# hyperplane-lab/ACL-GAN

Measured on AMD Instinct MI355X. Metric: training images/sec at 256x256 (gen+dis step), higher is better.
Workload: dtype fp32

## Files before the change

### acl-gan_amd/csrc/conv_fast.hip

```cpp
#include "conv_fast_common.h"
#include <cstring>

namespace aclgan {
namespace {


constexpr int BK = 16;
constexpr int WG_MAX_CHUNK = 1024 + 16;
constexpr int LDK = BK + 4;

template <int T, bool KC>
__device__ __forceinline__ void read_frags(const float* __restrict__ tile, int ld, int base, int lane, float (&f)[T][8]) {
    const int l31 = lane & 31, kh = lane >> 5;
    if (KC) {
#pragma unroll
        for (int t = 0; t < T; ++t) {
            const f32x4* p = reinterpret_cast<const f32x4*>(tile + (base + t * 32 + l31) * LDK + kh * 8);
            const f32x4 a = p[0], b = p[1];
            f[t][0] = a.x; f[t][1] = a.y; f[t][2] = a.z; f[t][3] = a.w;
            f[t][4] = b.x; f[t][5] = b.y; f[t][6] = b.z; f[t][7] = b.w;
        }
    } else {
#pragma unroll
        for (int ks = 0; ks < 8; ++ks)
// ... 275 lines not shown
        const int n = n0 + nc * 4;
        bo[i] = krow * p.k * p.k * p.Ci + (n < p.Ci ? n : 0);
    }
    const int cpt = p.Co >> 4;
    int aoff[A_IT];
    f32x4 ra[A_IT], rb[B_IT];
    float za[A_IT];
    int f_tap = -1, tapoff = 0;

    auto fetch = [&](int kt) __attribute__((always_inline)) {
        const int tq = kt / cpt, cc = kt - tq * cpt;
        if (tq != f_tap) {
            f_tap = tq;
            const int t = compact ? tap_list[tq] : tq;
            const int ty = t / Tx, tx = t - ty * Tx;
            tapoff = ((cy + p.s * ty) * p.k + (cx + p.s * tx)) * p.Ci;
#pragma unroll
            for (int i = 0; i < A_IT; ++i) {
                const int oy = ay[i] - ty, ox = ax[i] - tx;
                const bool ok = (unsigned)oy < (unsigned)p.Ho && (unsigned)ox < (unsigned)p.Wo;
                bool okk = ok;
                if (p.band > 0) okk = ok && (oy < 2 || oy >= p.Ho - 2 || ox < 2 || ox >= p.Wo - 2);
                const int dpix = p.dyv ? (ab[i] * p.Hf + 2 * (oy + 1) + p.py) * p.Wf + 2 * (ox + 1) + p.px
                                       : (ab[i] * p.Ho + oy) * p.Wo + ox;
                aoff[i] = okk ? dpix * p.Co + q * 4 : -1;
            }
        }
#pragma unroll
        for (int i = 0; i < A_IT; ++i) {
            ra[i] = *reinterpret_cast<const f32x4*>(p.dy + (size_t)(aoff[i] < 0 ? 0 : aoff[i]) + cc * 16);
            za[i] = aoff[i] < 0 ? 0.f : 1.f;
        }
#pragma unroll
        for (int i = 0; i < B_IT; ++i)
            if ((BK * NVB) % NT == 0 || tid + i * NT < BK * NVB)
                rb[i] = *reinterpret_cast<const f32x4*>(p.w + (size_t)bo[i] + tapoff + (size_t)cc * 16 * p.k * p.k * p.Ci);
    };
    auto stage = [&](int buf, bool real) __attribute__((always_inline)) {
        float* a = As + buf * BM * LDK;
        float* b = Bs + buf * BK * LDB;
#pragma unroll
        for (int i = 0; i < A_IT; ++i) *reinterpret_cast<f32x4*>(a + (r0 + i * RP) * LDK + q * 4) = ra[i] * za[i];
#pragma unroll
        for (int i = 0; i < B_IT; ++i) {
            const int idx = tid + i * NT;
            if ((BK * NVB) % NT == 0 || idx < BK * NVB) {
                const int krow = idx / NVB, nc = idx - krow * NVB;
                *reinterpret_cast<f32x4*>(b + krow * LDB + nc * 4) = rb[i];
            }
        }
    };

    f32x16 acc[TM][TN];
#pragma unroll
    for (int i = 0; i < TM; ++i)
#pragma unroll
        for (int j = 0; j < TN; ++j)
#pragma unroll
            for (int r = 0; r < 16; ++r) acc[i][j][r] = 0.f;

    const int nk_all = ntap * cpt;
    const int nkz = (nk_all + p.ksplit - 1) / p.ksplit;
    const int kbeg = slice * nkz, nk = min(nkz, nk_all - kbeg);
    if (nk <= 0) return;
    ACL_GEMM_MAINLOOP(TM, TN, true, false, kbeg, nk, As, Bs, BM * LDK, BK * LDB, LDK, LDB, wm * TM * 32, wn * TN * 32);

    const int l31 = lane & 31, lh = lane >> 5;
#pragma unroll
    for (int j = 0; j < TN; ++j) {
        const int n = n0 + wn * TN * 32 + j * 32 + l31;
        if (n >= p.Ci) continue;
#pragma unroll
        for (int i = 0; i < TM; ++i) {
#pragma unroll
            for (int r = 0; r < 16; ++r) {
                const int of = ri_o[wm * TM * 32 + i * 32 + (r & 3) + 8 * (r >> 2) + 4 * lh];
                if (of >= 0) {
                    float* o = p.dxp + (size_t)of * p.Ci + n;
                    if (p.ksplit > 1 || (p.mode == 2 && !p.ringpad)) atomicAdd(o, acc[i][j][r]);
                    else if (p.accumulate) *o += acc[i][j][r];
                    else *o = acc[i][j][r];
                }
            }
        }
    }
}

template <int WM, int WN, int TM, int TN>
int launch_dgrad_fast(const ConvGeom& g, DgFP p, hipStream_t st) {
    constexpr int BM = WM * TM * 32, BN = WN * TN * 32;
    int mmax = 0;
    for (int cy = 0; cy < g.s; ++cy)
        for (int cx = 0; cx < g.s; ++cx) {
            const int ylo = g.p > cy ? (g.p - cy + g.s - 1) / g.s : 0, xlo = g.p > cx ? (g.p - cx + g.s - 1) / g.s : 0;
            const int yhi = std::min(p.Hc - 1, (g.p + g.Hi - 1 - cy) / g.s), xhi = std::min(p.Wc - 1, (g.p + g.Wi - 1 - cx) / g.s);
            int inner = (yhi - ylo + 1) * (xhi - xlo + 1);
            if (p.band > 0) inner = std::max(0, p.Hc - 2 * p.band) * std::max(0, p.Wc - 2 * p.band);
            const int rows = p.mode == 0 ? p.Hc * p.Wc : (p.mode == 1 ? inner : p.Hc * p.Wc - inner);
            mmax = std::max(mmax, g.B * rows);
        }
    if (mmax <= 0) return ACLGAN_OK;
    p.Mc = mmax;
    p.tiles_n = cdiv(g.Ci, BN);
    p.nwg = cdiv(p.Mc, BM) * p.tiles_n;
    const int nk_min = ((g.k + g.s - 1) / g.s) * ((g.k + g.s - 1) / g.s) * (g.Co / 16);
    const int nblk = p.nwg * g.s * g.s;
    p.ksplit = 1;
    const int nk_plan = (p.mode == 2 && p.band == 0) ? std::max(g.Co / 16, nk_min / ((g.k + g.s - 1) / g.s)) : nk_min;
    if (nblk < 128 && nk_plan >= 32 && !sw(SW_DETERMINISTIC) && !p.ringpad)
        p.ksplit = max(1, min(nk_plan / 8, 512 / nblk));
    if (p.ksplit > 1 && p.mode == 0) {
        hipError_t e = hipMemsetAsync(p.dxp, 0, conv_dgrad_scratch_bytes(g), st);
        if (e != hipSuccess) return hip_fail(e, "memset dxp");
    }
    if (p.ksplit > 1 && p.mode == 1 && !p.accumulate) {
        hipError_t e = hipMemsetAsync(p.dxp, 0, (size_t)g.B * g.Hi * g.Wi * g.Ci * sizeof(float), st);
        if (e != hipSuccess) return hip_fail(e, "memset dx");
    }
    hipLaunchKernelGGL((conv_dgrad_fast_kernel<WM, WN, TM, TN>), dim3(p.nwg, 1, g.s * g.s * p.ksplit), dim3(WM * WN * 64), 0, st, p);
    ACL_CHECK_LAUNCH("conv_dgrad_fast_kernel");
    return ACLGAN_OK;
}

template <int WM, int WN, int TM, int TN>
int launch_dgrad_halo(const ConvGeom& g, DgFP p, hipStream_t st) {
    if (p.band == 0 && !p.ringpad && g.k == 3 && g.s == 1 && g.Ci % 128 == 0 && WM == 2 && WN == 2 && TM == 2 && TN == 2)
        return launch_dgrad_fast<2, 2, 1, 2>(g, p, st);
    return launch_dgrad_fast<WM, WN, TM, TN>(g, p, st);
}

template <int WM, int WN, int TM, int TN>
int dgrad_fast_all(const ConvGeom& g, DgFP p, float* dxp, float* dx, int accumulate, bool* direct, hipStream_t st) {
    if (g.up == 0 && dx != nullptr && (!sw(SW_DETERMINISTIC) || g.p == 0 || (dxp && conv_wino_ok(g)))) {
        *direct = true;
        p.dxp = dx; p.accumulate = accumulate;
        p.mode = 1;
        int rc = (dxp && conv_wino_ok(g)) ? conv_dgrad_wino_interior(g, p.dy, p.w, dx, accumulate, dxp, st)
             : (dxp && conv_s2k4_wino_ok(g, 1)) ? conv_dgrad_s2k4_wino_interior(g, p.dy, p.w, dx, accumulate, dxp, st)
                                      : launch_dgrad_fast<WM, WN, TM, TN>(g, p, st);
        if (rc) return rc;
        if (g.p > 0 && sw(SW_DETERMINISTIC)) {
            hipError_t e = hipMemsetAsync(dxp, 0, (size_t)g.B * g.Hp * g.Wp * g.Ci * sizeof(float), st);
            if (e != hipSuccess) return hip_fail(e, "memset padded grid");
            p.mode = 2; p.ringpad = 1; p.dxp = dxp; p.accumulate = 0;
            rc = launch_dgrad_fast<WM, WN, TM, TN>(g, p, st);
            if (rc) return rc;
            return conv_fold(g, dxp, dx, 1, st);
        }
        if (g.p > 0) { p.mode = 2; rc = launch_dgrad_halo<WM, WN, TM, TN>(g, p, st); }
        return rc;
    }
    *direct = false;
    p.dxp = dxp; p.mode = 0; p.accumulate = 0;
    return launch_dgrad_fast<WM, WN, TM, TN>(g, p, st);
}


template <int WM, int WN, int TM, int TN, bool ST>
__global__ void __launch_bounds__(WM * WN * 64) conv_wgrad_fast_kernel(WgFP p) {
    constexpr int BM = WM * TM * 32, BN = WN * TN * 32, NT = WM * WN * 64;
    constexpr int LDA = BM + 4, LDB = BN + 4, MVA = BM / 4, NVB = BN / 4;
    constexpr int A_IT = (BK * MVA + NT - 1) / NT, B_IT = (BK * NVB + NT - 1) / NT;
    __shared__ __attribute__((aligned(16))) float smem[2 * BK * (LDA + LDB)];
    float* As = smem;
    float* Bs = smem + 2 * BK * LDA;

    const int tid = threadIdx.x, lane = tid & 63, wave = tid >> 6;
    const int wm = wave / WN, wn = wave % WN;
    const int tile = xcd_map(blockIdx.x, p.nwg);
    const int m0 = (tile / p.tiles_n) * BM, n0 = (tile % p.tiles_n) * BN;
    const int pbeg = blockIdx.z * p.chunk;
    const int pend = min(p.P, pbeg + p.chunk);
    if (pbeg >= pend) return;
    const int phase = p.phases ? (int)blockIdx.y : 0;
    float* dwbase = p.dw + (size_t)phase * p.Co * p.Kn + (size_t)blockIdx.z * p.dw_zs;
    const int py = phase >> 1, px = phase & 1;

    __shared__ int4 pinfo[WG_MAX_CHUNK];
    const int st_tap = n0 / p.Ci, st_ky = st_tap / p.k, st_kx = st_tap - st_ky * p.k;
    for (int i = tid; i < pend - pbeg + BK; i += NT) {
        int b, oy, ox;
        wg_coord(p, min(pbeg + i, pend - 1), b, oy, ox);
        const int dyp = p.phases ? (b * p.Hf + 2 * (oy + 1) + py) * p.Wf + 2 * (ox + 1) + px : (b * p.Ho + oy) * p.Wo + ox;
        if (ST) {
            const int iy = refl(oy * p.s - p.p + st_ky, p.Hu) >> p.up, ix = refl(ox * p.s - p.p + st_kx, p.Wu) >> p.up;
            pinfo[i] = make_int4(b * p.Hi * p.Wi + iy * p.Wi + ix, 0, 0, dyp);
        } else {
            pinfo[i] = make_int4(oy * p.s - p.p, ox * p.s - p.p, b * p.Hi * p.Wi, dyp);
        }
    }
    __syncthreads();

    int a_m[A_IT], a_kr[A_IT];
#pragma unroll
    for (int i = 0; i < A_IT; ++i) {
        const int idx = tid + i * NT;
        a_kr[i] = idx / MVA;
        const int m = m0 + (idx - a_kr[i] * MVA) * 4;
        a_m[i] = m < p.Co ? m : 0;
    }
    int b_kr[B_IT], b_ci[B_IT], b_ky[B_IT], b_kx[B_IT];
#pragma unroll
    for (int i = 0; i < B_IT; ++i) {
        const int idx = tid + i * NT;
        b_kr[i] = idx / NVB;
        int n = n0 + (idx - b_kr[i] * NVB) * 4;
        if (n >= p.Kn) n = 0;
        const int tap = n / p.Ci;
        b_ci[i] = n - tap * p.Ci; b_ky[i] = tap / p.k; b_kx[i] = tap - b_ky[i] * p.k;
    }
    f32x4 ra[A_IT], rb[B_IT];
    float za[A_IT];
    const bool do_bias = p.db != nullptr && (tile % p.tiles_n) == 0;
    f32x4 bsum[A_IT];
#pragma unroll
    for (int i = 0; i < A_IT; ++i) bsum[i] = (f32x4){0.f, 0.f, 0.f, 0.f};

    auto fetch = [&](int kt) __attribute__((always_inline)) {
        const int pb = kt * BK;
#pragma unroll
        for (int i = 0; i < A_IT; ++i) {
            if ((BK * MVA) % NT != 0 && tid + i * NT >= BK * MVA) continue;
            const int pi = pb + a_kr[i];
            ra[i] = *reinterpret_cast<const f32x4*>(p.dy + (size_t)pinfo[pi].w * p.Co + a_m[i]);
            za[i] = pbeg + pi < pend ? 1.f : 0.f;
        }
#pragma unroll
        for (int i = 0; i < B_IT; ++i) {
            if ((BK * NVB) % NT != 0 && tid + i * NT >= BK * NVB) continue;
            if (ST) {
                rb[i] = *reinterpret_cast<const f32x4*>(p.x + (size_t)pinfo[pb + b_kr[i]].x * p.Ci + b_ci[i]);
            } else {
                const int4 pi = pinfo[pb + b_kr[i]];
                const int iy = refl(pi.x + b_ky[i], p.Hu) >> p.up;
                const int ix = refl(pi.y + b_kx[i], p.Wu) >> p.up;
                rb[i] = *reinterpret_cast<const f32x4*>(p.x + (size_t)(pi.z + iy * p.Wi + ix) * p.Ci + b_ci[i]);
            }
        }
    };
    auto stage = [&](int buf, bool real) __attribute__((always_inline)) {
        float* a = As + buf * BK * LDA;
        float* b = Bs + buf * BK * LDB;
#pragma unroll
        for (int i = 0; i < A_IT; ++i) {
            const int idx = tid + i * NT;
            if ((BK * MVA) % NT == 0 || idx < BK * MVA) {
                const f32x4 v = ra[i] * za[i];
                *reinterpret_cast<f32x4*>(a + a_kr[i] * LDA + (idx - a_kr[i] * MVA) * 4) = v;
                bsum[i] += v * (real ? 1.f : 0.f);
            }
        }
#pragma unroll
        for (int i = 0; i < B_IT; ++i) {
            const int idx = tid + i * NT;
            if ((BK * NVB) % NT == 0 || idx < BK * NVB) *reinterpret_cast<f32x4*>(b + b_kr[i] * LDB + (idx - b_kr[i] * NVB) * 4) = rb[i];
        }
    };

    f32x16 acc[TM][TN];
#pragma unroll
    for (int i = 0; i < TM; ++i)
#pragma unroll
        for (int j = 0; j < TN; ++j)
#pragma unroll
            for (int r = 0; r < 16; ++r) acc[i][j][r] = 0.f;

    ACL_GEMM_MAINLOOP(TM, TN, false, false, 0, (pend - pbeg + BK - 1) / BK, As, Bs, BK * LDA, BK * LDB, LDA, LDB, wm * TM * 32, wn * TN * 32);

    if (do_bias) {
        float* red = smem;
#pragma unroll
        for (int i = 0; i < A_IT; ++i) {
            const int idx = tid + i * NT;
            if ((BK * MVA) % NT == 0 || idx < BK * MVA) *reinterpret_cast<f32x4*>(red + a_kr[i] * BM + (idx - a_kr[i] * MVA) * 4) = bsum[i];
        }
        __syncthreads();
        if (tid < BM && m0 + tid < p.Co) {
            float t = 0.f;
#pragma unroll
            for (int r = 0; r < BK; ++r) t += red[r * BM + tid];
            atomicAdd(p.db + (size_t)blockIdx.z * p.db_zs + m0 + tid, t);
        }
    }
    const int l31 = lane & 31, lh = lane >> 5;
#pragma unroll
    for (int j = 0; j < TN; ++j) {
        const int n = n0 + wn * TN * 32 + j * 32 + l31;
        if (n >= p.Kn) continue;
#pragma unroll
        for (int i = 0; i < TM; ++i) {
#pragma unroll
            for (int r = 0; r < 16; ++r) {
                const int m = m0 + wm * TM * 32 + i * 32 + (r & 3) + 8 * (r >> 2) + 4 * lh;
                if (m < p.Co) {
                    atomicAdd(dwbase + (size_t)m * p.Kn + n, acc[i][j][r]);
                }
            }
        }
    }
}

constexpr int WGKC_TARGET = 768;

template <int WM, int WN, int TM, int TN>
__global__ void __launch_bounds__(WM * WN * 64) conv_wgrad_kc_kernel(WgFP pk, WgPartX xp) {
    constexpr int BM = WM * TM * 32, BN = WN * TN * 32, NT = WM * WN * 64;
    WgFP p = pk;
    if (pk.fsl) {
        const long long f = blockIdx.y;
        p.x += (pk.fsx_mod ? f % pk.fsx_mod : f) * pk.fs_x; p.dy += f * pk.fs_dy;
    }
    static_assert(BM % 64 == 0 && BN % 64 == 0 && BM + BN <= NT, "one staging unit (4 channels x 4 pixels) per thread, wave-uniform roles");
    constexpr int CH = 1024;
    __shared__ __attribute__((aligned(16))) float smem[2 * (BM + BN) * LDK];
    __shared__ int2 pinfo[CH + BK];
    float* As = smem;
    float* Bs = smem + 2 * BM * LDK;

    const int tid = threadIdx.x, lane = tid & 63, wave = tid >> 6;
    const int wm = wave / WN, wn = wave % WN;
    const int tile = xcd_map(blockIdx.x, p.nwg);
    const int m0 = (tile / p.tiles_n) * BM, n0 = (tile % p.tiles_n) * BN;
    const int pbeg = blockIdx.z * p.chunk;
    const int pend = min(p.P, pbeg + p.chunk);
    const int phase = (p.phases || p.fsl) ? (int)blockIdx.y : 0;
    float* dwbase = p.dw + (size_t)phase * p.Co * p.Kn;
    const int py = phase >> 1, px = phase & 1;
    const int st_tap = n0 / p.Ci, st_ky = st_tap / p.k, st_kx = st_tap - st_ky * p.k;

    const bool isA = tid < BM, isB = !isA && tid < BM + BN;
    const int u = isA ? tid : tid - BM;
    const int ncg = (isA ? BM : BN) >> 2;
    const int cg = u % ncg, pg = u / ncg;
    const float* src = isA ? p.dy : p.x;
    const int cstride = isA ? p.Co : p.Ci;
    const int chan = isA ? m0 + 4 * cg : (n0 - st_tap * p.Ci) + 4 * cg;
    float* mytile = isA ? As : Bs;
    const int tstride = (isA ? BM : BN) * LDK;
    f32x4 rr[4];
    float zm[4];
    const bool do_bias = p.db != nullptr && (tile % p.tiles_n) == 0;
    f32x4 bsum = {0.f, 0.f, 0.f, 0.f};

    f32x16 acc[TM][TN];
#pragma unroll
    for (int i = 0; i < TM; ++i)
#pragma unroll
        for (int j = 0; j < TN; ++j)
#pragma unroll
            for (int r = 0; r < 16; ++r) acc[i][j][r] = 0.f;

    for (int cb = pbeg; cb < pend; cb += CH) {
        const int ce = min(pend, cb + CH);
        for (int i = tid; i < ce - cb + BK; i += NT) {
            int b, oy, ox;
            wg_coord(p, min(cb + i, ce - 1), b, oy, ox);
            const int dyp = p.phases ? (b * p.Hf + 2 * (oy + 1) + py) * p.Wf + 2 * (ox + 1) + px : (b * p.Ho + oy) * p.Wo + ox;
            const int iy = refl(oy * p.s - p.p + st_ky, p.Hu) >> p.up, ix = refl(ox * p.s - p.p + st_kx, p.Wu) >> p.up;
            pinfo[i] = make_int2(b * p.Hi * p.Wi + iy * p.Wi + ix, dyp);
        }
        __syncthreads();

        auto fetch = [&](int kt) __attribute__((always_inline)) {
            const int pb = kt * BK + 4 * pg;
            if (isA || isB) {
#pragma unroll
                for (int j = 0; j < 4; ++j) {
                    const int2 pi = pinfo[pb + j];
                    rr[j] = *reinterpret_cast<const f32x4*>(src + (size_t)(isA ? pi.y : pi.x) * cstride + chan);
                    zm[j] = cb + pb + j < ce ? 1.f : 0.f;
                }
            }
        };
        auto stage = [&](int buf, bool real) __attribute__((always_inline)) {
            if (isA || isB) {
                float* t = mytile + buf * tstride;
                f32x4 v[4];
#pragma unroll
                for (int j = 0; j < 4; ++j) v[j] = rr[j] * zm[j];
                if (isA) {
                    const float on = real ? 1.f : 0.f;
#pragma unroll
                    for (int j = 0; j < 4; ++j) bsum += v[j] * on;
                }
#pragma unroll
                for (int c = 0; c < 4; ++c) {
                    const f32x4 k4 = {v[0][c], v[1][c], v[2][c], v[3][c]};
                    *reinterpret_cast<f32x4*>(t + (c * ncg + cg) * LDK + 4 * pg) = k4;
                }
            }
        };
        ACL_GEMM_MAINLOOP(TM, TN, true, true, 0, (ce - cb + BK - 1) / BK, As, Bs, BM * LDK, BN * LDK, LDK, LDK, wm * TM * 32, wn * TN * 32);
    }

    const bool partial = xp.part != nullptr;
    if (do_bias) {
        float* red = smem;
        if (isA) *reinterpret_cast<f32x4*>(red + pg * BM + 4 * cg) = bsum;
        __syncthreads();
        if (tid < BM) {
            const float t = red[tid] + red[BM + tid] + red[2 * BM + tid] + red[3 * BM + tid];
            if (partial) xp.part_b[((size_t)blockIdx.z * xp.ny + phase) * p.Co + m0 + tid] = t;
            else p.db[m0 + tid] += t;
        }
    }
    const int l31 = lane & 31, lh = lane >> 5;
    constexpr int MQ = BM / 4, NQ = BN / 4;
    if (partial) {
        float* pt = xp.part + (((size_t)blockIdx.z * xp.ny + phase) * p.nwg + tile) * (BM * BN);
#pragma unroll
        for (int j = 0; j < TN; ++j)
#pragma unroll
            for (int i = 0; i < TM; ++i)
#pragma unroll
                for (int r = 0; r < 16; ++r) {
                    const int rw = wm * TM * 32 + i * 32 + (r & 3) + 8 * (r >> 2) + 4 * lh;
                    pt[rw * BN + wn * TN * 32 + j * 32 + l31] = acc[i][j][r];
                }
        return;
    }
#pragma unroll
    for (int j = 0; j < TN; ++j) {
        const int cr = wn * TN * 32 + j * 32 + l31;
        const int n = n0 + 4 * (cr % NQ) + cr / NQ;
#pragma unroll
        for (int i = 0; i < TM; ++i) {
#pragma unroll
            for (int r = 0; r < 16; ++r) {
                const int rw = wm * TM * 32 + i * 32 + (r & 3) + 8 * (r >> 2) + 4 * lh;
                const int m = m0 + 4 * (rw % MQ) + rw / MQ;
                dwbase[(size_t)m * p.Kn + n] += acc[i][j][r];
            }
        }
    }
}

bool wgrad_kc_ok(const ConvGeom& g) {
    return !sw(SW_NOWGKC) && g.Co % 64 == 0 && g.Ci % 64 == 0;
}

template <int WM, int WN, int TM, int TN>
int launch_wgrad_kc(const ConvGeom& g, WgFP p, void* part, hipStream_t st) {
    constexpr int BM = WM * TM * 32, BN = WN * TN * 32;
    const int ny = p.fsl ? p.fsl : (p.phases ? 4 : 1);
    const WgPlan q = wgrad_plan(g.Co, p.Ci, p.Kn, p.P, ny, BK, WGKC_TARGET);
    if (q.BM != BM || q.BN != BN) { set_error("wgrad_kc: tile plan mismatch"); return ACLGAN_EINVAL; }
    p.tiles_n = q.tiles_n; p.nwg = q.nwg; p.chunk = q.chunk;
    WgPartX xp;
    xp.ny = ny; xp.part = nullptr; xp.part_b = nullptr;
    const bool use_part = q.splits > 1 || ny > 1;
    if (use_part) {
        if (!part) { set_error("wgrad_kc: %d slices need the scratch buffer", q.splits); return ACLGAN_EINVAL; }
        xp.part = (float*)part;
        xp.part_b = xp.part + (size_t)q.splits * ny * q.nwg * BM * BN;
    }
    hipLaunchKernelGGL((conv_wgrad_kc_kernel<WM, WN, TM, TN>), dim3(p.nwg, ny, q.splits), dim3(WM * WN * 64), 0, st, p, xp);
    ACL_CHECK_LAUNCH("conv_wgrad_kc_kernel");
    if (use_part) {
        const int64_t n = (int64_t)ny * g.Co * (p.Kn / 4);
        hipLaunchKernelGGL(wgrad_finish_kernel, dim3((int)std::min<int64_t>(cdiv64(n, 256), 4096)), dim3(256), 0, st, p, xp, BM, BN, q.splits);
        ACL_CHECK_LAUNCH("wgrad_finish_kernel");
    }
    return ACLGAN_OK;
}
int launch_wgrad_kc_any(const ConvGeom& g, const WgFP& p, void* part, hipStream_t st) {
    if (g.Co % 128 == 0 && p.Ci % 128 == 0) return launch_wgrad_kc<2, 2, 2, 2>(g, p, part, st);
    if (g.Co % 128 == 0) return launch_wgrad_kc<2, 2, 2, 1>(g, p, part, st);
    if (p.Ci % 128 == 0) return launch_wgrad_kc<2, 2, 1, 2>(g, p, part, st);
    return launch_wgrad_kc<2, 2, 1, 1>(g, p, part, st);
}

template <int WM, int WN, int TM, int TN>
int launch_wgrad_fast(const ConvGeom& g, WgFP p, hipStream_t st, void* det_part = nullptr) {
    constexpr int BM = WM * TM * 32, BN = WN * TN * 32;
    p.tiles_n = cdiv(p.Kn, BN);
    p.nwg = cdiv(g.Co, BM) * p.tiles_n;
    const int target = 1536;
    const int ny = p.phases ? 4 : 1;
    int splits = max(1, target / (p.nwg * ny));
    splits = max(1, min(splits, cdiv(p.P, 256)));
    splits = max(splits, cdiv(p.P, 1024));
    p.chunk = cdiv(cdiv(p.P, splits), 16) * 16;
    splits = cdiv(p.P, p.chunk);
    float* dw_out = p.dw; float* db_out = p.db;
    const int64_t ndw = (int64_t)ny * g.Co * p.Kn;
    if (det_part != nullptr && splits > 1) {
        hipError_t e = hipMemsetAsync(det_part, 0, (size_t)splits * (ndw + g.Co) * sizeof(float), st);
        if (e != hipSuccess) return hip_fail(e, "memset wgrad slices");
        p.dw = (float*)det_part; p.dw_zs = ndw;
        if (p.db) { p.db = (float*)det_part + (size_t)splits * ndw; p.db_zs = g.Co; }
    }
    if (p.Ci % BN == 0) hipLaunchKernelGGL((conv_wgrad_fast_kernel<WM, WN, TM, TN, true>), dim3(p.nwg, ny, splits), dim3(WM * WN * 64), 0, st, p);
    else hipLaunchKernelGGL((conv_wgrad_fast_kernel<WM, WN, TM, TN, false>), dim3(p.nwg, ny, splits), dim3(WM * WN * 64), 0, st, p);
    ACL_CHECK_LAUNCH("conv_wgrad_fast_kernel");
    if (p.dw_zs) {
        int rc = reduce_slices_ordered(p.dw, ndw, splits, dw_out, st);
        if (rc) return rc;
        if (db_out) { rc = reduce_slices_ordered(p.db, g.Co, splits, db_out, st); if (rc) return rc; }
    }
    return ACLGAN_OK;
}
size_t wgrad_fast_det_bytes(const ConvGeom& g, int Kn, int P, int ny) {
    const int nwg = cdiv(g.Co, 128) * cdiv(Kn, 128);
    int splits = std::max(1, 1536 / (nwg * ny));
    splits = std::max(1, std::min(splits, cdiv(P, 256)));
    splits = std::max(splits, cdiv(P, 1024)) + 1;
    return (size_t)splits * ((size_t)ny * g.Co * Kn + g.Co) * sizeof(float) + 256;
}


template <int WM, int WN, int TM, int TN>
int up5_fwd_t(const ConvGeom& g, const float* x, const float* w, const float* bias, float* y, float* wp, hipStream_t st, float* keepV) {
    const int64_t nm = (int64_t)4 * g.Co * 9 * (g.Ci / 4);
    if (!(conv_up5_wino_ok(g) && wino_u_cached(w, conv_up5_wino_u_variant(g, 0, keepV != nullptr)))) {
        hipLaunchKernelGGL(up5_merge_kernel, dim3((int)std::min<int64_t>(cdiv64(nm, 256), 2048)), dim3(256), 0, st, w, wp, g.Co, g.Ci);
        ACL_CHECK_LAUNCH("up5_merge_kernel");
    }
    FwdFP p;
    p.fsl = 0; p.fsx_mod = 0; p.fs_x = p.fs_w = p.fs_y = 0; p.w16 = nullptr; p.x16 = nullptr;
    p.x = x; p.w = wp; p.bias = bias; p.y = y;
    p.Hi = g.Hi; p.Wi = g.Wi; p.Ci = g.Ci; p.Ho = g.Hi - 2; p.Wo = g.Wi - 2; p.Co = g.Co; p.k = 3; p.s = 1; p.p = 0;
    p.up = 0; p.Hu = g.Hi; p.Wu = g.Wi; p.M = g.B * p.Ho * p.Wo; p.K = 9 * g.Ci; p.act = g.act; p.tiles_n = 0; p.nwg = 0; p.nkz = 0;
    p.B = g.B; p.ring = 0; p.phases = 1; p.Hf = g.Ho; p.Wf = g.Wo; p.part = nullptr; p.rows = 0;
    ConvGeom gp = g;
    gp.M = p.M; gp.K = p.K;
    char* wino_scr = (char*)wp + up5_merged_bytes(g) + ((fwd_partial_bytes(g, 2, BK) + 255) & ~(size_t)255);
    if (keepV && !conv_up5_wino_ok(g)) { set_error("conv_fwd: this layer does not keep a Winograd input transform"); return ACLGAN_EINVAL; }
    int rc = conv_up5_wino_ok(g) ? conv_up5_wino_fwd_phases(g, x, wp, bias, y, wino_scr, st, keepV, w) : launch_fwd_fast<WM, WN, TM, TN>(gp, p, st);
    if (rc) return rc;
    p.w = w;
    p.Hi = g.Hi; p.Wi = g.Wi; p.Ho = g.Ho; p.Wo = g.Wo; p.k = 5; p.s = 1; p.p = 2; p.up = 1; p.Hu = g.Hu; p.Wu = g.Wu;
    p.M = g.M; p.K = g.K; p.ring = 2; p.phases = 0;
    p.part = (float*)((char*)wp + up5_merged_bytes(g));
    return launch_fwd_fast<WM, WN, TM, TN>(g, p, st);
}

template <int WM, int WN, int TM, int TN>
int up5_wgrad_t(const ConvGeom& g, const float* x, const float* dy, float* dw, float* db, float* dwp, hipStream_t st, const float* haveV) {
    const size_t nb = (size_t)4 * g.Co * 9 * g.Ci * sizeof(float);
    hipError_t e = hipMemsetAsync(dwp, 0, nb, st);
    if (e != hipSuccess) return hip_fail(e, "memset dwp");
    const bool kc = wgrad_kc_ok(g);
    void* part = (char*)dwp + up5_dwp_bytes(g);
    WgFP p;
    p.fsl = 0; p.fsx_mod = 0; p.fs_x = p.fs_dy = 0;
    p.x = x; p.dy = dy; p.dw = dwp; p.db = db;
    p.Hi = g.Hi; p.Wi = g.Wi; p.Ci = g.Ci; p.Ho = g.Hi - 2; p.Wo = g.Wi - 2; p.Co = g.Co; p.k = 3; p.s = 1; p.p = 0;
    p.up = 0; p.Hu = g.Hi; p.Wu = g.Wi; p.P = g.B * p.Ho * p.Wo; p.Kn = 9 * g.Ci; p.chunk = 0; p.tiles_n = 0; p.nwg = 0;
    p.B = g.B; p.ring = 0; p.phases = 1; p.Hf = g.Ho; p.Wf = g.Wo;
    int rc;
    if (kc && conv_up5_wino_wgrad_scratch_bytes(g)) {
        void* wino_scr = (char*)dwp + ((wgrad_part_scratch(g, BK, WGKC_TARGET) + 255) & ~(size_t)255);
        rc = conv_up5_wino_wgrad_phases(g, x, dy, dwp, db, wino_scr, st, haveV);
    } else rc = kc ? launch_wgrad_kc_any(g, p, part, st) : launch_wgrad_fast<WM, WN, TM, TN>(g, p, st);
    if (rc) return rc;
    const int64_t ns = (int64_t)g.Co * 25 * (g.Ci / 4);
    hipLaunchKernelGGL(up5_scatter_kernel, dim3((int)std::min<int64_t>(cdiv64(ns, 256), 2048)), dim3(256), 0, st, dwp, dw, g.Co, g.Ci);
    ACL_CHECK_LAUNCH("up5_scatter_kernel");
    p.dw = dw;
    p.Hi = g.Hi; p.Wi = g.Wi; p.Ho = g.Ho; p.Wo = g.Wo; p.k = 5; p.s = 1; p.p = 2; p.up = 1; p.Hu = g.Hu; p.Wu = g.Wu;
    p.ring = 2; p.phases = 0; p.Kn = g.K;
    p.P = g.B * (g.Ho * g.Wo - (g.Ho - 4) * (g.Wo - 4));
    return kc ? launch_wgrad_kc_any(g, p, part, st) : launch_wgrad_fast<WM, WN, TM, TN>(g, p, st);
}

template <int WM, int WN, int TM, int TN>
int up5_dgrad_t(const ConvGeom& g, const float* dy, const float* w, float* dx, int accumulate, float* wp, hipStream_t st) {
    const int64_t nm = (int64_t)4 * g.Co * 9 * (g.Ci / 4);
    if (!(conv_up5_wino_ok(g) && wino_u_cached(w, conv_up5_wino_u_variant(g, 1, false)))) {
        hipLaunchKernelGGL(up5_merge_kernel, dim3((int)std::min<int64_t>(cdiv64(nm, 256), 2048)), dim3(256), 0, st, w, wp, g.Co, g.Ci);
        ACL_CHECK_LAUNCH("up5_merge_kernel");
    }
    ConvGeom gv = g;
    gv.k = 3; gv.s = 1; gv.p = 0; gv.up = 0; gv.Hu = g.Hi; gv.Wu = g.Wi; gv.Hp = g.Hi; gv.Wp = g.Wi;
    gv.Ho = g.Hi - 2; gv.Wo = g.Wi - 2; gv.M = g.B * gv.Ho * gv.Wo; gv.K = 9 * g.Ci;
    DgFP p;
    p.dy = dy; p.dxp = dx;
    p.Ho = gv.Ho; p.Wo = gv.Wo; p.Co = g.Co; p.Ci = g.Ci; p.k = 3; p.s = 1; p.Hp = g.Hi; p.Wp = g.Wi;
    p.Hc = g.Hi; p.Wc = g.Wi; p.Mc = 0; p.tiles_n = 0; p.nwg = 0; p.ksplit = 1;
    p.mode = 1; p.pad = 0; p.B = g.B; p.Hi = g.Hi; p.Wi = g.Wi;
    p.dyv = 1; p.Hf = g.Ho; p.Wf = g.Wo; p.band = 0; p.upshift = 0; p.Hd = g.Hi; p.Wd = g.Wi;
    if (conv_up5_wino_ok(g)) {
        const int rc = conv_up5_wino_dgrad_phases(g, dy, wp, dx, accumulate, (char*)wp + up5_merged_bytes(g), st, w);
        if (rc) return rc;
    } else for (int ph = 0; ph < 4; ++ph) {
        p.w = wp + (size_t)ph * g.Co * 9 * g.Ci;
        p.py = ph >> 1; p.px = ph & 1;
        p.accumulate = (ph > 0 || accumulate) ? 1 : 0;
        const int rc = launch_dgrad_fast<WM, WN, TM, TN>(gv, p, st);
        if (rc) return rc;
    }
    p.w = w;
    p.Ho = g.Ho; p.Wo = g.Wo; p.k = 5; p.s = 1; p.Hp = g.Hp; p.Wp = g.Wp; p.Hc = g.Hp; p.Wc = g.Wp;
    p.mode = 2; p.accumulate = 1; p.pad = 2; p.Hi = g.Hu; p.Wi = g.Wu;
    p.dyv = 0; p.band = 6; p.upshift = 1; p.Hd = g.Hi; p.Wd = g.Wi;
    if (sw(SW_DETERMINISTIC)) {
        float* dxp = (float*)((char*)wp + up5_merged_bytes(g));
        hipError_t e = hipMemsetAsync(dxp, 0, (size_t)g.B * g.Hp * g.Wp * g.Ci * sizeof(float), st);
        if (e != hipSuccess) return hip_fail(e, "memset padded grid");
        p.ringpad = 1; p.dxp = dxp; p.accumulate = 0;
        const int rc = launch_dgrad_fast<WM, WN, TM, TN>(g, p, st);
        if (rc) return rc;
        return conv_fold(g, dxp, dx, 1, st);
    }
    return launch_dgrad_fast<WM, WN, TM, TN>(g, p, st);
}


}

size_t conv_up5_scratch_bytes(const ConvGeom& g) {
    return up5_eligible(g) ? (size_t)4 * g.Co * 9 * g.Ci * sizeof(float) : 0;
}
size_t conv_up5_dgrad_scratch_bytes(const ConvGeom& g) {
    if (sw(SW_NOFAST) || !up5_eligible(g)) return 0;
    const size_t padded = sw(SW_DETERMINISTIC) ? (size_t)g.B * g.Hp * g.Wp * g.Ci * sizeof(float) : 0;
    return up5_merged_bytes(g) + std::max(conv_up5_wino_dgrad_scratch_bytes(g), padded);
}
size_t conv_wgrad_fast_scratch_bytes(const ConvGeom& g) {
    if (sw(SW_NOFAST)) return 0;
    if (wgrad_kc_ok(g) && conv_wino_ok(g)) return conv_wgrad_wino_scratch_bytes(g);
    if (wgrad_kc_ok(g)) return ((wgrad_part_scratch(g, BK, WGKC_TARGET) + 255) & ~(size_t)255) + (up5_eligible(g) ? conv_up5_wino_wgrad_scratch_bytes(g) : 0);
    if (sw(SW_DETERMINISTIC)) return wgrad_fast_det_bytes(g, g.K, g.M, 1);
    return conv_up5_scratch_bytes(g);
}
size_t conv_fwd_fast_scratch_bytes(const ConvGeom& g) {
    if (sw(SW_NOFAST)) return 0;
    if (conv_wino_ok(g)) return conv_wino_scratch_bytes(g);
    if (up5_eligible(g)) return up5_merged_bytes(g) + ((fwd_partial_bytes(g, 2, BK) + 255) & ~(size_t)255) + conv_up5_wino_fwd_scratch_bytes(g);
    return std::max(fwd_partial_bytes(g, 0, BK), conv_s2k4_wino_scratch_bytes(g));
}

int conv_up5_fwd(const ConvGeom& g, const float* x, const float* w, const float* bias, float* y, void* scratch, hipStream_t st, float* keepV) {
    if (sw(SW_NOFAST) || !up5_eligible(g) || !scratch) return ACLGAN_EUNSUPPORTED;
    if (g.Co > 64) return up5_fwd_t<2, 2, 2, 2>(g, x, w, bias, y, (float*)scratch, st, keepV);
    if (g.Co > 32) return up5_fwd_t<4, 1, 2, 2>(g, x, w, bias, y, (float*)scratch, st, keepV);
    return up5_fwd_t<4, 1, 2, 1>(g, x, w, bias, y, (float*)scratch, st, keepV);
}

int conv_up5_dgrad(const ConvGeom& g, const float* dy, const float* w, float* dx, int accumulate, void* scratch, hipStream_t st) {
    if (sw(SW_NOFAST) || !up5_eligible(g) || !scratch) return ACLGAN_EUNSUPPORTED;
    if (sw(SW_NOUP5DGRAD)) return ACLGAN_EUNSUPPORTED;
    if (g.Ci > 64) return up5_dgrad_t<2, 2, 2, 2>(g, dy, w, dx, accumulate, (float*)scratch, st);
    if (g.Ci > 32) return up5_dgrad_t<4, 1, 2, 2>(g, dy, w, dx, accumulate, (float*)scratch, st);
    return up5_dgrad_t<4, 1, 2, 1>(g, dy, w, dx, accumulate, (float*)scratch, st);
}

int conv_up5_wgrad(const ConvGeom& g, const float* x, const float* dy, float* dw, float* db, void* scratch, hipStream_t st, const float* haveV) {
    if (sw(SW_NOFAST) || !up5_eligible(g) || !scratch || !dw) return ACLGAN_EUNSUPPORTED;
    if (sw(SW_DETERMINISTIC) && !wgrad_kc_ok(g)) return ACLGAN_EUNSUPPORTED;
    if (g.Co > 64) return up5_wgrad_t<2, 2, 2, 2>(g, x, dy, dw, db, (float*)scratch, st, haveV);
    if (g.Co > 32) return up5_wgrad_t<2, 2, 1, 2>(g, x, dy, dw, db, (float*)scratch, st, haveV);
    return up5_wgrad_t<1, 4, 1, 2>(g, x, dy, dw, db, (float*)scratch, st, haveV);
}

int gemm_slices_f32(const float* A, const float* Bm, float* Cm, int T, int K, int N, int nslices, int a_mod, hipStream_t st) {
    if (K % 16 != 0 || T <= 0 || N <= 0) { set_error("gemm_slices_f32: bad shape"); return ACLGAN_EINVAL; }
    FwdFP p;
    p.part = nullptr; p.rows = 0; p.w16 = nullptr; p.x16 = nullptr;
    p.x = A; p.w = Bm; p.bias = nullptr; p.y = Cm;
    p.Hi = T; p.Wi = 1; p.Ci = K; p.Ho = T; p.Wo = 1; p.Co = N; p.k = 1; p.s = 1; p.p = 0;
    p.up = 0; p.Hu = T; p.Wu = 1; p.M = T; p.K = K; p.act = ACLGAN_ACT_NONE; p.tiles_n = 0; p.nwg = 0; p.nkz = K / BK;
    p.B = 1; p.ring = 0; p.phases = 0; p.Hf = 0; p.Wf = 0;
    p.fsl = nslices; p.fsx_mod = a_mod; p.fs_x = (long long)T * K; p.fs_w = (long long)N * K; p.fs_y = (long long)T * N;
    if (N > 64) {
        p.tiles_n = cdiv(N, 128); p.nwg = cdiv(T, 64) * p.tiles_n;
        hipLaunchKernelGGL((conv_fwd_fast_kernel<2, 2, 1, 2, 4>), dim3(p.nwg, nslices, 1), dim3(256), 0, st, p);
    } else if (N > 32) {
        p.tiles_n = cdiv(N, 64); p.nwg = cdiv(T, 256) * p.tiles_n;
        hipLaunchKernelGGL((conv_fwd_fast_kernel<4, 1, 2, 2>), dim3(p.nwg, nslices, 1), dim3(256), 0, st, p);
    } else {
        p.tiles_n = cdiv(N, 32); p.nwg = cdiv(T, 256) * p.tiles_n;
        hipLaunchKernelGGL((conv_fwd_fast_kernel<4, 1, 2, 1>), dim3(p.nwg, nslices, 1), dim3(256), 0, st, p);
    }
    ACL_CHECK_LAUNCH("conv_fwd_fast_kernel(gemm slices)");
    return ACLGAN_OK;
}

int conv_fwd_stats_chunk(const ConvGeom& g) {
    if (sw(SW_NOSTATFUSE) || sw(SW_NOFAST) || g.Ci % 16 != 0 || g.act != ACLGAN_ACT_NONE) return 0;
    if (conv_wino_ok(g)) return 16;
    return (g.Ho % 4 == 0 && g.Wo % 4 == 0 && conv_s2k4_wino_ok(g, 0)) ? 16 : 0;
}
size_t conv_fwd_keep_bytes(const ConvGeom& g) {
    if (sw(SW_NOKEEPV) || sw(SW_NOFAST) || !wgrad_kc_ok(g)) return 0;
    if (up5_eligible(g)) return conv_up5_wino_wgrad_scratch_bytes(g) ? conv_up5_wino_keep_bytes(g) : 0;
    if (g.Ci % 16 != 0 || !conv_wino_ok(g) || !conv_wgrad_wino_scratch_bytes(g)) return 0;
    return conv_wino_keep_bytes(g);
}
int conv_fwd_fast(const ConvGeom& g, const float* x, const float* w, const float* bias, float* y, hipStream_t st, void* scratch, float* stats, float* keepV) {
    if (sw(SW_NOFAST) || g.Ci % 16 != 0) return ACLGAN_EUNSUPPORTED;
    if (scratch && conv_wino_ok(g)) return conv_fwd_wino(g, x, w, bias, y, scratch, st, stats, keepV);
    if (scratch && !keepV && conv_s2k4_wino_ok(g, 0) && (!stats || (g.Ho % 4 == 0 && g.Wo % 4 == 0)))
        return conv_fwd_s2k4_wino(g, x, w, bias, y, scratch, st, stats);
    if (stats || keepV) return ACLGAN_EUNSUPPORTED;
    FwdFP p;
    p.fsl = 0; p.fsx_mod = 0; p.fs_x = p.fs_w = p.fs_y = 0; p.w16 = nullptr; p.x16 = nullptr;
    p.part = (float*)scratch; p.rows = 0;
    p.x = x; p.w = w; p.bias = bias; p.y = y;
    p.Hi = g.Hi; p.Wi = g.Wi; p.Ci = g.Ci; p.Ho = g.Ho; p.Wo = g.Wo; p.Co = g.Co; p.k = g.k; p.s = g.s; p.p = g.p;
    p.up = g.up; p.Hu = g.Hu; p.Wu = g.Wu; p.M = g.M; p.K = g.K; p.act = g.act; p.tiles_n = 0; p.nwg = 0; p.nkz = 0;
    p.B = g.B; p.ring = 0; p.phases = 0; p.Hf = 0; p.Wf = 0;
    if (g.Co > 64) return launch_fwd_fast<2, 2, 2, 2>(g, p, st);
    if (g.Co > 32) return launch_fwd_fast<4, 1, 2, 2>(g, p, st);
    return launch_fwd_fast<4, 1, 2, 1>(g, p, st);
}

int conv_dgrad_fast(const ConvGeom& g, const float* dy, const float* w, float* dxp, float* dx, int accumulate, bool* direct, hipStream_t st) {
    *direct = false;
    if (sw(SW_NOFAST) || g.Co % 16 != 0 || g.Ci % 4 != 0) return ACLGAN_EUNSUPPORTED;
    if (sw(SW_NODIRECT)) dx = nullptr;
    if (sw(SW_DETERMINISTIC) && !dxp) { set_error("conv_dgrad: deterministic mode needs the scratch buffer"); return ACLGAN_EINVAL; }
    DgFP p;
    p.dy = dy; p.w = w; p.dxp = dxp;
    p.Ho = g.Ho; p.Wo = g.Wo; p.Co = g.Co; p.Ci = g.Ci; p.k = g.k; p.s = g.s; p.Hp = g.Hp; p.Wp = g.Wp;
    p.Hc = cdiv(g.Hp, g.s); p.Wc = cdiv(g.Wp, g.s); p.Mc = 0; p.tiles_n = 0; p.nwg = 0; p.ksplit = 1;
    p.mode = 0; p.accumulate = 0; p.pad = g.p; p.B = g.B; p.Hi = g.Hu; p.Wi = g.Wu;
    p.dyv = 0; p.py = 0; p.px = 0; p.Hf = 0; p.Wf = 0; p.band = 0; p.upshift = 0; p.Hd = g.Hu; p.Wd = g.Wu;
    if (g.Ci > 64) return dgrad_fast_all<2, 2, 2, 2>(g, p, dxp, dx, accumulate, direct, st);
    if (g.Ci > 32) return dgrad_fast_all<4, 1, 2, 2>(g, p, dxp, dx, accumulate, direct, st);
    return dgrad_fast_all<4, 1, 2, 1>(g, p, dxp, dx, accumulate, direct, st);
}

size_t gemm_at_b_slices_scratch(int T, int M, int N, int nslices) {
    return wgrad_partial_bytes(wgrad_plan(M, N, N, T, nslices, BK, WGKC_TARGET), M, nslices) + 256;
}
int gemm_at_b_slices_f32(const float* A, const float* Bm, float* Cm, int T, int M, int N, int nslices, int b_mod, void* part, hipStream_t st) {
    if (M % 64 != 0 || N % 64 != 0 || T <= 0) { set_error("gemm_at_b_slices_f32: bad shape"); return ACLGAN_EINVAL; }
    WgFP p;
    p.x = Bm; p.dy = A; p.dw = Cm; p.db = nullptr;
    p.Hi = T; p.Wi = 1; p.Ci = N; p.Ho = T; p.Wo = 1; p.Co = M; p.k = 1; p.s = 1; p.p = 0;
    p.up = 0; p.Hu = T; p.Wu = 1; p.P = T; p.Kn = N; p.chunk = 0; p.tiles_n = 0; p.nwg = 0;
    p.B = 1; p.ring = 0; p.phases = 0; p.Hf = 0; p.Wf = 0;
    p.fsl = nslices; p.fsx_mod = b_mod; p.fs_x = (long long)T * N; p.fs_dy = (long long)T * M;
    p.dw_overwrite = 1;
    ConvGeom g;
    memset(&g, 0, sizeof g);
    g.Co = M; g.Ci = N;
// ... 71 lines not shown
```

Baseline: 97.34.

## Hand-pipeline wgrad KC mainloop with masked tail and full-grid XCD remap

Replaces the generic GEMM mainloop macro in the channel-contiguous weight-gradient kernel with a hand-written double-buffered loop. The next tile's global fetch and LDS staging are interleaved between the first and remaining MFMA steps, with a scheduling barrier between them. Zero-masking now applies only to the last tile, and the bias-accumulation branch is specialized at compile time. The XCD block remapping now covers the whole (x,y,z) grid rather than just blockIdx.x, which spreads phase and split slices across dies. The cost is more code duplication and higher register pressure, and the schedule barrier could hurt MFMA issue order.

```diff
diff --git a/acl-gan_amd/csrc/conv_fast.hip b/acl-gan_amd/csrc/conv_fast.hip
--- a/acl-gan_amd/csrc/conv_fast.hip
+++ b/acl-gan_amd/csrc/conv_fast.hip
@@ -601,12 +601,75 @@
 
 constexpr int WGKC_TARGET = 768;
 
+#define ACL_WGKC_TILE_MFMA_1_7                                                                           \
+    mfma_step<TM, TN>(fa, fb, 1, acc); mfma_step<TM, TN>(fa, fb, 2, acc); mfma_step<TM, TN>(fa, fb, 3, acc); mfma_step<TM, TN>(fa, fb, 4, acc); \
+    mfma_step<TM, TN>(fa, fb, 5, acc); mfma_step<TM, TN>(fa, fb, 6, acc); mfma_step<TM, TN>(fa, fb, 7, acc)
+#define ACL_WGKC_SLICE(BIAS_)                                                                            \
+    for (int cb = pbeg; cb < pend; cb += CH) {                                                           \
+        const int ce = min(pend, cb + CH);                                                               \
+        for (int i = tid; i < ce - cb + BK; i += NT) {       \
+            int b, oy, ox;                                                                               \
+            wg_coord(p, min(cb + i, ce - 1), b, oy, ox);                                                 \
+            const int dyp = p.phases ? (b * p.Hf + 2 * (oy + 1) + py) * p.Wf + 2 * (ox + 1) + px : (b * p.Ho + oy) * p.Wo + ox; \
+            const int iy = refl(oy * p.s - p.p + st_ky, p.Hu) >> p.up, ix = refl(ox * p.s - p.p + st_kx, p.Wu) >> p.up; \
+            pinfo[i] = make_int2(b * p.Hi * p.Wi + iy * p.Wi + ix, dyp);                                 \
+        }                                                                                                \
+        __syncthreads();                                                                                 \
+        const int nk = (ce - cb + BK - 1) / BK;                                                          \
+        float zm[4], zp[4];       \
+        _Pragma("unroll") for (int j = 0; j < 4; ++j) {                                                  \
+            zm[j] = cb + (nk - 1) * BK + 4 * pg + j < ce ? 1.f : 0.f;                                    \
+            zp[j] = nk == 1 ? zm[j] : 1.f;                                                               \
+        }                                                                                                \
+        fetch(0);                                                                                        \
+        stage_masked(0, zp, BIAS_);                                                                      \
+        fetch(min(1, nk - 1));                                                                           \
+        __syncthreads();                                                                                 \
+        int kt = 0;                                                                                      \
+        for (; kt < nk - 2; ++kt) {                                                                      \
+            const int cur = kt & 1;                                                                      \
+            float fa[TM][8], fb[TN][8];                                                                  \
+            read_frags<TM, true>(As + cur * BM * LDK, LDK, wm * TM * 32, lane, fa);                      \
+            read_frags<TN, true>(Bs + cur * BN * LDK, LDK, wn * TN * 32, lane, fb);                      \
+            mfma_step<TM, TN>(fa, fb, 0, acc);                                                           \
+            stage_plain(cur ^ 1, BIAS_);                                                                 \
+            fetch(kt + 2);                                                                               \
+            __builtin_amdgcn_sched_barrier(0x6);    \
+            ACL_WGKC_TILE_MFMA_1_7;                                                                        \
+            __syncthreads();                                                                             \
+        }                                                                                                \
+        if (kt == nk - 2) {                                                           \
+            const int cur = kt & 1;                                                                      \
+            float fa[TM][8], fb[TN][8];                                                                  \
+            read_frags<TM, true>(As + cur * BM * LDK, LDK, wm * TM * 32, lane, fa);                      \
+            read_frags<TN, true>(Bs + cur * BN * LDK, LDK, wn * TN * 32, lane, fb);                      \
+            mfma_step<TM, TN>(fa, fb, 0, acc);                                                           \
+            stage_masked(cur ^ 1, zm, BIAS_);                                                            \
+            __builtin_amdgcn_sched_barrier(0x6);                                                         \
+            ACL_WGKC_TILE_MFMA_1_7;                                                                        \
+            __syncthreads();                                                                             \
+            ++kt;                                                                                        \
+        }                                                                                                \
+        {                                                                                                \
+            const int cur = kt & 1;                                                                      \
+            float fa[TM][8], fb[TN][8];                                                                  \
+            read_frags<TM, true>(As + cur * BM * LDK, LDK, wm * TM * 32, lane, fa);                      \
+            read_frags<TN, true>(Bs + cur * BN * LDK, LDK, wn * TN * 32, lane, fb);                      \
+            mfma_step<TM, TN>(fa, fb, 0, acc); ACL_WGKC_TILE_MFMA_1_7;                                                  \
+            __syncthreads();                     \
+        }                                                                                                \
+    }
+
 template <int WM, int WN, int TM, int TN>
 __global__ void __launch_bounds__(WM * WN * 64) conv_wgrad_kc_kernel(WgFP pk, WgPartX xp) {
     constexpr int BM = WM * TM * 32, BN = WN * TN * 32, NT = WM * WN * 64;
+    const int nyz = (int)gridDim.y;
+    const int vid = xcd_map(blockIdx.x + pk.nwg * (blockIdx.y + nyz * blockIdx.z), pk.nwg * nyz * (int)gridDim.z);
+    const int tile = vid % pk.nwg, vyz = vid / pk.nwg;
+    const int by = vyz % nyz, bz = vyz / nyz;
     WgFP p = pk;
     if (pk.fsl) {
-        const long long f = blockIdx.y;
+        const long long f = by;
         p.x += (pk.fsx_mod ? f % pk.fsx_mod : f) * pk.fs_x; p.dy += f * pk.fs_dy;
     }
     static_assert(BM % 64 == 0 && BN % 64 == 0 && BM + BN <= NT, "one staging unit (4 channels x 4 pixels) per thread, wave-uniform roles");
@@ -618,11 +681,10 @@
 
     const int tid = threadIdx.x, lane = tid & 63, wave = tid >> 6;
     const int wm = wave / WN, wn = wave % WN;
-    const int tile = xcd_map(blockIdx.x, p.nwg);
     const int m0 = (tile / p.tiles_n) * BM, n0 = (tile % p.tiles_n) * BN;
-    const int pbeg = blockIdx.z * p.chunk;
+    const int pbeg = bz * p.chunk;
     const int pend = min(p.P, pbeg + p.chunk);
-    const int phase = (p.phases || p.fsl) ? (int)blockIdx.y : 0;
+    const int phase = (p.phases || p.fsl) ? by : 0;
     float* dwbase = p.dw + (size_t)phase * p.Co * p.Kn;
     const int py = phase >> 1, px = phase & 1;
     const int st_tap = n0 / p.Ci, st_ky = st_tap / p.k, st_kx = st_tap - st_ky * p.k;
@@ -637,7 +699,6 @@
     float* mytile = isA ? As : Bs;
     const int tstride = (isA ? BM : BN) * LDK;
     f32x4 rr[4];
-    float zm[4];
     const bool do_bias = p.db != nullptr && (tile % p.tiles_n) == 0;
     f32x4 bsum = {0.f, 0.f, 0.f, 0.f};
 
@@ -649,48 +710,46 @@
 #pragma unroll
             for (int r = 0; r < 16; ++r) acc[i][j][r] = 0.f;
 
-    for (int cb = pbeg; cb < pend; cb += CH) {
-        const int ce = min(pend, cb + CH);
-        for (int i = tid; i < ce - cb + BK; i += NT) {
-            int b, oy, ox;
-            wg_coord(p, min(cb + i, ce - 1), b, oy, ox);
-            const int dyp = p.phases ? (b * p.Hf + 2 * (oy + 1) + py) * p.Wf + 2 * (ox + 1) + px : (b * p.Ho + oy) * p.Wo + ox;
-            const int iy = refl(oy * p.s - p.p + st_ky, p.Hu) >> p.up, ix = refl(ox * p.s - p.p + st_kx, p.Wu) >> p.up;
-            pinfo[i] = make_int2(b * p.Hi * p.Wi + iy * p.Wi + ix, dyp);
-        }
-        __syncthreads();
-
-        auto fetch = [&](int kt) __attribute__((always_inline)) {
-            const int pb = kt * BK + 4 * pg;
-            if (isA || isB) {
-#pragma unroll
-                for (int j = 0; j < 4; ++j) {
-                    const int2 pi = pinfo[pb + j];
-                    rr[j] = *reinterpret_cast<const f32x4*>(src + (size_t)(isA ? pi.y : pi.x) * cstride + chan);
-                    zm[j] = cb + pb + j < ce ? 1.f : 0.f;
-                }
-            }
-        };
-        auto stage = [&](int buf, bool real) __attribute__((always_inline)) {
-            if (isA || isB) {
-                float* t = mytile + buf * tstride;
-                f32x4 v[4];
-#pragma unroll
-                for (int j = 0; j < 4; ++j) v[j] = rr[j] * zm[j];
-                if (isA) {
-                    const float on = real ? 1.f : 0.f;
-#pragma unroll
-                    for (int j = 0; j < 4; ++j) bsum += v[j] * on;
-                }
-#pragma unroll
-                for (int c = 0; c < 4; ++c) {
-                    const f32x4 k4 = {v[0][c], v[1][c], v[2][c], v[3][c]};
-                    *reinterpret_cast<f32x4*>(t + (c * ncg + cg) * LDK + 4 * pg) = k4;
-                }
-            }
-        };
-        ACL_GEMM_MAINLOOP(TM, TN, true, true, 0, (ce - cb + BK - 1) / BK, As, Bs, BM * LDK, BN * LDK, LDK, LDK, wm * TM * 32, wn * TN * 32);
-    }
+    auto fetch = [&](int kt) __attribute__((always_inline)) {
+        const int pb = kt * BK + 4 * pg;
+        if (isA || isB) {
+#pragma unroll
+            for (int j = 0; j < 4; ++j) {
+                const int2 pi = pinfo[pb + j];
+                rr[j] = *reinterpret_cast<const f32x4*>(src + (size_t)(isA ? pi.y : pi.x) * cstride + chan);
+            }
+        }
+    };
+    auto transpose_store = [&](int buf, const f32x4 (&v)[4]) __attribute__((always_inline)) {
+        float* t = mytile + buf * tstride;
+#pragma unroll
+        for (int c = 0; c < 4; ++c) {
+            const f32x4 k4 = {v[0][c], v[1][c], v[2][c], v[3][c]};
+            *reinterpret_cast<f32x4*>(t + (c * ncg + cg) * LDK + 4 * pg) = k4;
+        }
+    };
+    auto stage_plain = [&](int buf, bool bias) __attribute__((always_inline)) {
+        if (isA || isB) {
+            if (bias && isA) {
+#pragma unroll
+                for (int j = 0; j < 4; ++j) bsum += rr[j];
+            }
+            transpose_store(buf, rr);
+        }
+    };
+    auto stage_masked = [&](int buf, const float (&z)[4], bool bias) __attribute__((always_inline)) {
+        if (isA || isB) {
+            f32x4 v[4];
+#pragma unroll
+            for (int j = 0; j < 4; ++j) v[j] = rr[j] * z[j];
+            if (bias && isA) {
+#pragma unroll
+                for (int j = 0; j < 4; ++j) bsum += v[j];
+            }
+            transpose_store(buf, v);
+        }
+    };
+    if (do_bias) { ACL_WGKC_SLICE(true) } else { ACL_WGKC_SLICE(false) }
 
     const bool partial = xp.part != nullptr;
     if (do_bias) {
@@ -699,14 +758,14 @@
         __syncthreads();
         if (tid < BM) {
             const float t = red[tid] + red[BM + tid] + red[2 * BM + tid] + red[3 * BM + tid];
-            if (partial) xp.part_b[((size_t)blockIdx.z * xp.ny + phase) * p.Co + m0 + tid] = t;
+            if (partial) xp.part_b[((size_t)bz * xp.ny + phase) * p.Co + m0 + tid] = t;
             else p.db[m0 + tid] += t;
         }
     }
     const int l31 = lane & 31, lh = lane >> 5;
     constexpr int MQ = BM / 4, NQ = BN / 4;
     if (partial) {
-        float* pt = xp.part + (((size_t)blockIdx.z * xp.ny + phase) * p.nwg + tile) * (BM * BN);
+        float* pt = xp.part + (((size_t)bz * xp.ny + phase) * p.nwg + tile) * (BM * BN);
 #pragma unroll
         for (int j = 0; j < TN; ++j)
 #pragma unroll
@@ -733,6 +792,8 @@
         }
     }
 }
+#undef ACL_WGKC_SLICE
+#undef ACL_WGKC_TILE_MFMA_1_7
 
 bool wgrad_kc_ok(const ConvGeom& g) {
     return !sw(SW_NOWGKC) && g.Co % 64 == 0 && g.Ci % 64 == 0;
```

After: 97.44 (median of 3 runs). No clear change (+0.1%).
